# qianduoduolr/FGVC

Measured on AMD Instinct MI355X. Metric: frames/sec + ms/corr-volume, 480p 8-frame clip, 1/2/4/8 MI355X, higher is better.
Workload: dtype f16 + fp6 (e2m3) MFMA operands, f32 accumulate; top-k near-ties re-scored in f64 from f32 features

## Files before the change

### fgvc_amd/csrc/conv_split.hip

```cpp
#include "common.hpp"

namespace fgvc {

struct ConvSplitParams {
  const uint16_t* x;
  const uint16_t* w;
  const float* bias;
  const float* residual;
  uint16_t* y_split;
  float* y_f32;
  int N, H, W, Hp, Wp, Cin, Cout, relu;
  int n_ty, n_tx;
  int debug;
  float acc_scale;
  float out_scale;
  int out_fmt;
  int* overflow;
  const uint16_t* x2;
  const uint16_t* w2;
  int Cin2;
  unsigned char* y_bank;
  int bank_normalize;
  int bank_row_bytes;
};
// ... 730 lines not shown
__global__ __launch_bounds__(256) void normalize_nhwc_kernel(const float* __restrict__ in, float* __restrict__ out,
                                                              uint16_t* __restrict__ out_split, int C, int normalize,
                                                              long long npix) {
  const long long pixel = (long long)blockIdx.x * 4 + (threadIdx.x >> 6);
  const int lane = threadIdx.x & 63;
  if (pixel >= npix) return;
  const float* src = in + (size_t)pixel * C;
  float ss = 0.f;
  for (int c = lane * 4; c < C; c += 256) {
    const f32x4 v = *reinterpret_cast<const f32x4*>(src + c);
    ss += v.x * v.x + v.y * v.y + v.z * v.z + v.w * v.w;
  }
#pragma unroll
  for (int m = 32; m >= 1; m >>= 1) ss += __shfl_xor(ss, m);
  const float inv = normalize ? 1.0f / fmaxf(sqrtf(ss), 1e-12f) : 1.0f;
  for (int c = lane * 4; c < C; c += 256) {
    f32x4 v = *reinterpret_cast<const f32x4*>(src + c);
    v *= inv;
    if (out) *reinterpret_cast<f32x4*>(out + pixel * C + c) = v;
    if (out_split) {
      ushort4 hv, lv;
      if constexpr (FMT == 0) {
        split_bf16_4(v, hv, lv);
      } else {
        typedef _Float16 f16x4 __attribute__((ext_vector_type(4)));
        f16x4 h, l;
#pragma unroll
        for (int i = 0; i < 4; ++i) {
          const float xs = v[i] * 16384.f;
          h[i] = (_Float16)xs;
          l[i] = (_Float16)(xs - (float)h[i]);
        }
        hv = __builtin_bit_cast(ushort4, h);
        lv = __builtin_bit_cast(ushort4, l);
      }
      *reinterpret_cast<ushort4*>(out_split + pixel * 2 * C + c) = hv;
      *reinterpret_cast<ushort4*>(out_split + pixel * 2 * C + C + c) = lv;
    }
  }
}

__device__ __forceinline__ int n6_scale_exp(float m) {
  if (!(m > 0.f)) return -40;
  int e;
  const float f = frexpf(m * (1.0f / 7.5f), &e);
  int s = (f > 0.5f) ? e : e - 1;
  if (m * exp2f((float)-s) > 7.5f) ++s;
  return imax(s, -40);
}
__device__ __forceinline__ unsigned n6_code(float y) {
  const float a = fabsf(y);
  const float inv_step = a < 2.f ? 8.f : (a < 4.f ? 4.f : 2.f);
  const float r = fminf(__builtin_rintf(a * inv_step) / inv_step, 7.5f);
  const float c = r < 2.f ? 8.f * r : (r < 4.f ? 8.f + 4.f * r : 16.f + 2.f * r);
  return (unsigned)c | (y < 0.f ? 32u : 0u);
}
__global__ __launch_bounds__(256) void normalize_f16f6p_kernel(const float* __restrict__ in, unsigned char* __restrict__ out, int normalize,
                                                                long long npix, int rowb) {
  const long long pixel = (long long)blockIdx.x * 4 + (threadIdx.x >> 6);
  const int lane = threadIdx.x & 63;
  if (pixel >= npix) return;
  const float* src = in + (size_t)pixel * 256;
  float ss;
  {
#pragma clang fp contract(off)
    const f32x4 v = *reinterpret_cast<const f32x4*>(src + 4 * lane);
    const float xx = v.x * v.x, yy = v.y * v.y, zz = v.z * v.z, ww = v.w * v.w;
    ss = ((xx + yy) + zz) + ww;
  }
#pragma unroll
  for (int m = 32; m >= 1; m >>= 1) ss += __shfl_xor(ss, m);
  const float inv = normalize ? 1.0f / fmaxf(sqrtf(ss), 1e-12f) : 1.0f;
  f32x4 x = *reinterpret_cast<const f32x4*>(src + 4 * lane);
  x *= inv;
  unsigned char* row = out + (size_t)pixel * rowb;
  if (rowb > 1024) *reinterpret_cast<f32x4*>(row + 1024 + 16 * lane) = x;
  typedef _Float16 f16x4 __attribute__((ext_vector_type(4)));
  f16x4 hv;
  float hf[4], lf[4], mh = 0.f, ml = 0.f;
#pragma unroll
  for (int i = 0; i < 4; ++i) {
    const float xs = x[i] * 256.f;
    const _Float16 h = (_Float16)xs;
    hv[i] = h;
    hf[i] = (float)h;
    lf[i] = (xs - hf[i]) * 256.f;
    mh = fmaxf(mh, fabsf(hf[i]));
    ml = fmaxf(ml, fabsf(lf[i]));
  }
  *reinterpret_cast<f16x4*>(row + 8 * lane) = hv;
#pragma unroll
  for (int m = 1; m <= 8; m <<= 1) {
    if (m == 2) continue;
    mh = fmaxf(mh, __shfl_xor(mh, m));
    ml = fmaxf(ml, __shfl_xor(ml, m));
  }
  const int sh = n6_scale_exp(mh), sl = n6_scale_exp(ml);
  const float ih = exp2f((float)-sh), il = exp2f((float)-sl);
  unsigned ph = 0, pl = 0;
#pragma unroll
  for (int i = 0; i < 4; ++i) {
    ph |= n6_code(hf[i] * ih) << (6 * i);
    pl |= n6_code(lf[i] * il) << (6 * i);
  }
  const int v = lane >> 4, hi = (lane >> 1) & 1, pi = ((lane >> 2) & 3) * 2 + (lane & 1);
  const int w = pi < 6 ? pi : 0;
  const int pa = (4 * w) / 3, oa = 32 * w - 24 * pa;
  const int base = (lane & ~13) ;
  const int la = base + 4 * (pa >> 1) + (pa & 1), lb = base + 4 * ((pa + 1) >> 1) + ((pa + 1) & 1);
  const unsigned ha = __shfl(ph, la), hb = __shfl(ph, lb), qa = __shfl(pl, la), qb = __shfl(pl, lb);
  const unsigned wh = (ha >> oa) | (hb << (24 - oa)), wl = (qa >> oa) | (qb << (24 - oa));
  if (pi < 4) {
    *reinterpret_cast<unsigned*>(row + 512 + 32 * v + 16 * hi + 4 * pi) = wh;
    *reinterpret_cast<unsigned*>(row + 704 + 32 * v + 16 * hi + 4 * pi) = wl;
  } else if (pi < 6) {
    *reinterpret_cast<unsigned*>(row + 640 + 32 * (v >> 1) + 16 * hi + 8 * (v & 1) + 4 * (pi - 4)) = wh;
    *reinterpret_cast<unsigned*>(row + 832 + 32 * (v >> 1) + 16 * hi + 8 * (v & 1) + 4 * (pi - 4)) = wl;
  } else if (pi == 6) {
    row[896 + 16 * hi + v] = (unsigned char)(sh + 127 - 4);
  } else {
    row[896 + 16 * hi + 4 + v] = (unsigned char)(sl + 127 - 4);
  }
  if (lane < 2) *reinterpret_cast<unsigned long long*>(row + 904 + 16 * lane) = 0ull;
  else if (lane < 26) *reinterpret_cast<unsigned*>(row + 928 + 4 * (lane - 2)) = 0u;
}

static int g_conv_debug = 0;
void set_conv_debug(int v) { g_conv_debug = v; }
static int g_conv_narrow = 1;
void set_conv_narrow(int v) { g_conv_narrow = v; }
static int g_conv_cot_cap = 0;
void set_conv_cot_cap(int v) { g_conv_cot_cap = v; }

template <int COT, int OUT_FMT, bool RES, bool F32OUT, bool GENERIC, bool BANK = false, int CIN_TAG = 0>
__global__ __launch_bounds__(256, 1) void conv256p_kernel(ConvSplitParams p) {
  constexpr int NA = COT / 64, PPW = NA * 2;
  constexpr int TROWS = 8, PATCHB = (TROWS + 2) * CV_PW * 128, SLOTB = COT * 128, NPIECE = (TROWS + 2) * 5;
  __shared__ __attribute__((aligned(16))) unsigned char smem[PATCHB + 3 * SLOTB + COT * 4];
  unsigned char* patch = smem;
  unsigned char* wring = smem + PATCHB;
  float* bias_lds = reinterpret_cast<float*>(smem + PATCHB + 3 * SLOTB);
  const long long t_begin = __builtin_amdgcn_s_memtime();
  const int tid = threadIdx.x, lane = tid & 63;
  const int wave = __builtin_amdgcn_readfirstlane(tid >> 6);
  const int ch = wave & 1, pr = wave >> 1;
  const int n = lane & 31, h = lane >> 5;
  const int d_row = lane >> 3, d_slot = lane & 7;
  int bid = blockIdx.x;
  const int nimg = bid / (p.n_ty * p.n_tx);
  bid -= nimg * p.n_ty * p.n_tx;
  const int ty = bid / p.n_tx, tx = bid - ty * p.n_tx;
  const int y0 = ty * TROWS, x0 = tx * 32;
  const int co_base = blockIdx.y * COT;
  const int nchunk = p.Cin / 32;
  const uint32_t pixb = (uint32_t)nchunk * 128u;

  const uint32_t w_lane_off = (uint32_t)(d_row * 128 + ((d_slot ^ (d_row >> 1)) << 4));
  const uint32_t wo[2] = {w_lane_off, w_lane_off ^ 64u};
  const uint32_t ring_lds = lds_addr(wring), patch_lds = lds_addr(patch);
  const uint32_t wl = ring_lds + (uint32_t)((ch * (COT / 2) + n) * 128) + ((((uint32_t)h) ^ (uint32_t)((n >> 1) & 7)) << 4);
  uint32_t pl[3][2];
#pragma unroll
  for (int dx = 0; dx < 3; ++dx)
#pragma unroll
    for (int par = 0; par < 2; ++par) {
      const uint32_t key = (uint32_t)((((n + dx) >> 1) & 7) ^ (4 * par));
      pl[dx][par] = patch_lds + (uint32_t)((4 * pr * CV_PW + n + dx) * 128) + ((((uint32_t)h) ^ key) << 4);
    }
  const uint32_t pf_lane_off = (uint32_t)d_row * pixb + (uint32_t)((d_slot ^ (d_row >> 1)) << 4);
  const uint32_t lane16 = (uint32_t)lane * 16u;
  int ptab;
  {
    const int k = lane & 15, i = imin(wave + 4 * k, NPIECE - 1);
    const int prow = i / 5, pc0 = (i - prow * 5) * 8;
    const int goff = (int)((uint32_t)(prow * p.Wp + pc0) * pixb);
    const int ldst = (prow * CV_PW + pc0) * 128;
    const int key = ((prow + (pc0 >> 3)) & 1) << 6;
    ptab = lane < 16 ? goff : lane < 32 ? ldst : key;
  }
  const unsigned char* xb_tile = reinterpret_cast<const unsigned char*>(p.x) + (uint32_t)((nimg * p.Hp + y0) * p.Wp + x0) * pixb;
  const unsigned char* wb_tile = reinterpret_cast<const unsigned char*>(p.w) + (uint32_t)(co_base * 128);
  const uint32_t piece_off = (uint32_t)(wave * PPW * 1024);
  auto weight_base = [&](int chunk, int tap) { return wb_tile + (uint32_t)((tap * nchunk + chunk) * p.Cout * 128); };
  auto weight_piece = [&](const unsigned char* base, uint32_t dst, int j) {
    const unsigned char* src = base + piece_off + (uint32_t)(j * 1024);
    const uint32_t d = dst + piece_off + (uint32_t)(j * 1024);
    asm volatile("s_mov_b32 m0, %2\n\ts_nop 0\n\tglobal_load_lds_dwordx4 %0, %1" ::"v"(wo[j & 1]), "s"(src), "s"(d) : "memory");
  };

  if (tid < COT / 4) reinterpret_cast<f32x4*>(bias_lds)[tid] = reinterpret_cast<const f32x4*>(p.bias + co_base)[tid];
  for (int i = wave; i < NPIECE; i += 4) {
    const int prow = i / 5, pc0 = (i - prow * 5) * 8;
    const int P = prow * CV_PW + pc0 + d_row;
    const int sl = d_slot ^ ((P >> 1) & 7);
    const size_t gpix = ((size_t)nimg * p.Hp + (y0 + prow)) * p.Wp + (x0 + pc0 + d_row);
    conv_lds_dma_16(reinterpret_cast<const unsigned char*>(p.x) + gpix * pixb + sl * 16, lds_addr(patch + (prow * CV_PW + pc0) * 128));
  }
#pragma unroll
  for (int j = 0; j < PPW; ++j) weight_piece(weight_base(0, 0), ring_lds, j);
#pragma unroll
  for (int j = 0; j < PPW; ++j) weight_piece(weight_base(0, 1), ring_lds + SLOTB, j);

  __builtin_amdgcn_s_waitcnt(0x0F70);

  const long long t_loop0 = __builtin_amdgcn_s_memtime();
  {
    const size_t wb64 = (size_t)wb_tile, xb64 = (size_t)xb_tile;
    const int s_tap = __builtin_amdgcn_readfirstlane(nchunk * p.Cout * 128), s_chunk = __builtin_amdgcn_readfirstlane(p.Cout * 128);
    const int s_nchunk = __builtin_amdgcn_readfirstlane(nchunk), s_ring = __builtin_amdgcn_readfirstlane((int)ring_lds);
    const int s_patch = __builtin_amdgcn_readfirstlane((int)patch_lds), s_piece = __builtin_amdgcn_readfirstlane((int)piece_off);
    typedef int i32x2 __attribute__((ext_vector_type(2)));
    const i32x2 s_wb = {__builtin_amdgcn_readfirstlane((int)(uint32_t)wb64), __builtin_amdgcn_readfirstlane((int)(uint32_t)(wb64 >> 32))};
    const i32x2 s_xb = {__builtin_amdgcn_readfirstlane((int)(uint32_t)xb64), __builtin_amdgcn_readfirstlane((int)(uint32_t)(xb64 >> 32))};
    typedef int i32x2_t __attribute__((ext_vector_type(2)));
    i32x2_t loop_cycles;
    const int nchunk2 = p.x2 ? p.Cin2 / 32 : 0;
    const uint32_t pixb2 = (uint32_t)nchunk2 * 128u;
    const uint32_t pf_lane_off2 = (uint32_t)d_row * pixb2 + (uint32_t)((d_slot ^ (d_row >> 1)) << 4);
    int ptab2;
    {
      const int k2 = lane & 15, i2 = imin(wave + 4 * k2, NPIECE - 1);
      const int prow = i2 / 5, pc0 = (i2 - prow * 5) * 8;
      const int goff = (int)((uint32_t)(prow * p.Wp + pc0) * pixb2);
      ptab2 = lane < 16 ? goff : lane < 32 ? (prow * CV_PW + pc0) * 128 : (((prow + (pc0 >> 3)) & 1) << 6);
    }
    const size_t w2b64 = (size_t)p.w2 + (uint32_t)(co_base * 128), x2b64 = (size_t)p.x2 + (size_t)((uint32_t)((nimg * p.Hp + y0) * p.Wp + x0) * pixb2);
    const i32x2 s_w2b = {__builtin_amdgcn_readfirstlane((int)(uint32_t)w2b64), __builtin_amdgcn_readfirstlane((int)(uint32_t)(w2b64 >> 32))};
    const i32x2 s_x2b = {__builtin_amdgcn_readfirstlane((int)(uint32_t)x2b64), __builtin_amdgcn_readfirstlane((int)(uint32_t)(x2b64 >> 32))};
    const int s_last2 = __builtin_amdgcn_readfirstlane(nchunk2 ? nchunk - 1 : -1), s_nchunk2 = __builtin_amdgcn_readfirstlane(nchunk2);
#define C256P_INPUTS                                                                                                              \
  "{v232}"(wl), "{v233}"(pl[0][0]), "{v234}"(pl[0][1]), "{v235}"(pl[1][0]), "{v236}"(pl[1][1]), "{v237}"(pl[2][0]), "{v238}"(pl[2][1]),     \
      "{v239}"(wo[0]), "{v240}"(wo[1]), "{v241}"(pf_lane_off), "{v242}"(lane16), "{v243}"(ptab), "{v244}"(pf_lane_off2), "{v245}"(ptab2),  \
      "{s[20:21]}"(s_wb), "{s22}"(s_tap), "{s23}"(s_chunk), "{s[24:25]}"(s_xb), "{s26}"(s_nchunk), "{s27}"(s_ring), "{s28}"(s_patch),      \
      "{s29}"(s_piece), "{s46}"(s_last2), "{s[48:49]}"(s_w2b), "{s[50:51]}"(s_x2b), "{s52}"(s_nchunk2)
    if constexpr (COT == 256) {
#include "conv256p_loop.inc"
    } else {
#include "conv128p_loop.inc"
    }
#undef C256P_INPUTS
    if ((p.debug & 8) && blockIdx.x == 300 && blockIdx.y == 0 && lane == 0 && p.y_split) {
      long long* o = reinterpret_cast<long long*>(p.y_split) + wave * 8;
      o[4] = (long long)(uint32_t)loop_cycles.x | ((long long)loop_cycles.y << 32);
      o[5] = nchunk * 9 + nchunk2;
      o[0] = t_loop0 - t_begin;
    }
  }
  f32x16 acc[NA][4];
  if constexpr (NA == 4)
    asm volatile(""
                 : "={a[0:15]}"(acc[0][0]), "={a[16:31]}"(acc[0][1]), "={a[32:47]}"(acc[0][2]), "={a[48:63]}"(acc[0][3]), "={a[64:79]}"(acc[1][0]),
                   "={a[80:95]}"(acc[1][1]), "={a[96:111]}"(acc[1][2]), "={a[112:127]}"(acc[1][3]), "={a[128:143]}"(acc[NA - 2][0]),
                   "={a[144:159]}"(acc[NA - 2][1]), "={a[160:175]}"(acc[NA - 2][2]), "={a[176:191]}"(acc[NA - 2][3]), "={a[192:207]}"(acc[NA - 1][0]),
                   "={a[208:223]}"(acc[NA - 1][1]), "={a[224:239]}"(acc[NA - 1][2]), "={a[240:255]}"(acc[NA - 1][3]));
  else
    asm volatile(""
                 : "={a[0:15]}"(acc[0][0]), "={a[16:31]}"(acc[0][1]), "={a[32:47]}"(acc[0][2]), "={a[48:63]}"(acc[0][3]), "={a[64:79]}"(acc[1][0]),
                   "={a[80:95]}"(acc[1][1]), "={a[96:111]}"(acc[1][2]), "={a[112:127]}"(acc[1][3]));

  int lane_e;
  asm volatile("v_mbcnt_lo_u32_b32 %0, -1, 0\n\tv_mbcnt_hi_u32_b32 %0, -1, %0" : "=v"(lane_e));
  {
  int lane = lane_e, n = lane & 31, h = lane >> 5;
  int Wp_e = __builtin_amdgcn_readfirstlane(p.Wp);
  asm volatile("" : "+s"(Wp_e));
  constexpr int RPW = 4, CW = COT / 2, RB = CW * 4, RS = RB + 16, LPR = RB / 16, RPI = 64 / LPR;
  static_assert(4 * 32 * RS <= PATCHB + 3 * SLOTB, "epilogue staging");
  __syncthreads();
  long long ts0 = __builtin_amdgcn_s_memtime(), ts1 = 0, ts2 = 0, ts3 = 0, ts4 = 0;
  unsigned char* tile = smem + wave * (32 * RS);
  const int co_w = co_base + ch * CW;
  int mv_row = lane / LPR, mv_col = (lane % LPR) * 16;
  auto row_fence = [&]() { asm volatile("" : "+v"(n), "+v"(h), "+v"(mv_row), "+v"(mv_col)); };
  auto wave_sync = [&]() { asm volatile("s_waitcnt lgkmcnt(0)" ::: "memory"); };
  constexpr int RSLOTS = RB / 16, RPIECES = 32 * RB / 1024, RPPP = 1024 / RB;
  static_assert(4 * 32 * RS + 4 * 32 * RB <= PATCHB + 3 * SLOTB, "residual tiles");
  unsigned char* rtile = smem + 4 * (32 * RS) + wave * (32 * RB);
  const bool has_res = GENERIC || BANK ? p.residual != nullptr : RES;
  auto residual_dma = [&](int b_) {
    const int y_ = y0 + RPW * pr + b_;
    if (!has_res || b_ >= RPW || y_ >= p.H) return;
    const unsigned char* src = reinterpret_cast<const unsigned char*>(p.residual + (((size_t)nimg * p.H + y_) * p.W + x0) * p.Cout + co_w);
    const int pmax = p.W - 1 - x0;
#pragma unroll
    for (int j = 0; j < RPIECES; ++j) {
      const int pp = j * RPPP + (lane * 16) / RB, ps = ((lane * 16) % RB) / 16;
      const uint32_t voff = (uint32_t)(imin(pp, pmax) * p.Cout * 4 + ((ps ^ (pp & (RSLOTS - 1))) << 4));
      conv_lds_dma_16s(voff, src, lds_addr(rtile + j * 1024));
    }
  };
  auto residual_wait = [&](int stores_behind) {
    if (x0 + 32 > p.W || stores_behind == 0) asm volatile("s_waitcnt vmcnt(0)" ::: "memory");
    else if (stores_behind == 32 / RPI) asm volatile("s_waitcnt vmcnt(%0)" ::"n"(32 / RPI) : "memory");
    else asm volatile("s_waitcnt vmcnt(%0)" ::"n"(2 * (32 / RPI)) : "memory");
  };
  auto residual_at = [&](int cw) {
    return *reinterpret_cast<const f32x4*>(rtile + n * RB + ((((cw * 4) >> 4) ^ (n & (RSLOTS - 1))) << 4));
  };
  residual_dma(0);
  const bool tile_full = x0 + 32 <= p.W;
  auto store_rows = [&](unsigned char* dst) {
    unsigned char* d0 = dst + (size_t)mv_row * p.Cout * 4 + mv_col;
    const unsigned char* t0 = tile + mv_row * RS + mv_col;
    if (tile_full) {
#pragma unroll
      for (int i = 0; i < 32 / RPI; ++i) *reinterpret_cast<uint4*>(d0 + (size_t)(i * RPI) * p.Cout * 4) = *reinterpret_cast<const uint4*>(t0 + i * RPI * RS);
    } else {
#pragma unroll
      for (int i = 0; i < 32 / RPI; ++i)
        if (x0 + i * RPI + mv_row < p.W) *reinterpret_cast<uint4*>(d0 + (size_t)(i * RPI) * p.Cout * 4) = *reinterpret_cast<const uint4*>(t0 + i * RPI * RS);
    }
  };
  if constexpr (BANK) {
    {
      constexpr int BK_RS = 1024 + 16;
      static_assert(COT == 256 && 2 * 32 * BK_RS <= PATCHB + 3 * SLOTB, "bank staging");
      unsigned char* rows = smem + pr * (32 * BK_RS);
      float* part = reinterpret_cast<float*>(rows);
      long long bts[6] = {}, bt_begin = 0;
#pragma unroll
      for (int b = 0; b < RPW; ++b) {
        row_fence();
        const int y = y0 + RPW * pr + b;
        const bool row_ok = y < p.H;
        if (b == 1) bt_begin = __builtin_amdgcn_s_memtime();
        if (b == 2) bts[4] = __builtin_amdgcn_s_memtime();
        const size_t fpix0 = ((size_t)nimg * p.H + imin(y, p.H - 1)) * p.W + x0;
        if (has_res && row_ok) residual_wait(b == 0 || 32 / RPI != 16 ? 0 : (p.bank_row_bytes > 1024 ? 32 : 16));
        f32x4 v[NA][4];
#pragma unroll
        for (int a = 0; a < NA; ++a)
#pragma unroll
          for (int g = 0; g < 4; ++g) {
            const int cw = a * 32 + 8 * g + 4 * h;
            const f32x4 bv = *reinterpret_cast<const f32x4*>(bias_lds + ch * CW + cw);
            v[a][g] = {fmaf(acc[a][b][4 * g + 0], p.acc_scale, bv.x), fmaf(acc[a][b][4 * g + 1], p.acc_scale, bv.y),
                         fmaf(acc[a][b][4 * g + 2], p.acc_scale, bv.z), fmaf(acc[a][b][4 * g + 3], p.acc_scale, bv.w)};
            if (has_res && row_ok) v[a][g] += residual_at(cw);
            if (p.relu) {
              v[a][g].x = fmaxf(v[a][g].x, 0.f); v[a][g].y = fmaxf(v[a][g].y, 0.f);
              v[a][g].z = fmaxf(v[a][g].z, 0.f); v[a][g].w = fmaxf(v[a][g].w, 0.f);
            }
          }
        if (has_res) { wave_sync(); residual_dma(b + 1); }
        if (b == 1) bts[0] = __builtin_amdgcn_s_memtime();
        __syncthreads();
        float pp[NA][4];
        {
#pragma clang fp contract(off)
#pragma unroll
          for (int a = 0; a < NA; ++a)
#pragma unroll
            for (int g = 0; g < 4; ++g) {
              const float xx = v[a][g].x * v[a][g].x, yy = v[a][g].y * v[a][g].y, zz = v[a][g].z * v[a][g].z, ww = v[a][g].w * v[a][g].w;
              pp[a][g] = ((xx + yy) + zz) + ww;
              part[(ch * 16 + a * 4 + g) * 64 + lane] = pp[a][g];
            }
        }
        __syncthreads();
        float ss;
        {
          float t[NA][4];
#pragma unroll
          for (int a = 0; a < NA; ++a)
#pragma unroll
            for (int g = 0; g < 4; ++g) t[a][g] = pp[a][g] + part[((ch ^ 1) * 16 + a * 4 + g) * 64 + lane];
          float u[2][4], w4[4];
#pragma unroll
          for (int g = 0; g < 4; ++g) { u[0][g] = t[0][g] + t[2][g]; u[1][g] = t[1][g] + t[3][g]; }
#pragma unroll
          for (int g = 0; g < 4; ++g) w4[g] = u[0][g] + u[1][g];
          const float z0 = w4[0] + w4[2], z1 = w4[1] + w4[3];
          const float s1 = z0 + z1;
          ss = s1 + __shfl_xor(s1, 32);
        }
        __syncthreads();
        if (b == 1) bts[1] = __builtin_amdgcn_s_memtime();
        const float inv = p.bank_normalize ? 1.0f / fmaxf(sqrtf(ss), 1e-12f) : 1.0f;
        unsigned char* row = rows + n * BK_RS;
#pragma unroll
        for (int vl = 0; vl < 2; ++vl)
#pragma unroll
          for (int hi = 0; hi < 2; ++hi) {
            unsigned A_[16], B_[16];
            float mh = 0.f, ml = 0.f;
#pragma unroll
            for (int m = 0; m < 4; ++m) {
              const int a = 2 * vl + (m >> 1), g = hi + 2 * (m & 1);
              f32x4 x = v[a][g];
              x *= inv;
              typedef _Float16 f16x4 __attribute__((ext_vector_type(4)));
              f16x4 hv;
#pragma unroll
              for (int k = 0; k < 4; ++k) {
                const float xs = x[k] * 256.f;
                const _Float16 hh_ = (_Float16)xs;
                hv[k] = hh_;
                const float fh = (float)hh_, fl = (xs - fh) * 256.f;
                mh = fmaxf(mh, fabsf(fh)); ml = fmaxf(ml, fabsf(fl));
                A_[4 * m + k] = __builtin_bit_cast(unsigned, fh);
                B_[4 * m + k] = __builtin_bit_cast(unsigned, fl);
              }
              *reinterpret_cast<f16x4*>(row + 2 * (128 * ch + 32 * a + 8 * g + 4 * h)) = hv;
            }
#pragma unroll
            for (int j = 0; j < 16; ++j) {
              const auto t2 = __builtin_amdgcn_permlane32_swap(A_[j], B_[j], false, false);
              A_[j] = t2[0]; B_[j] = t2[1];
            }
            const auto tm = __builtin_amdgcn_permlane32_swap(__builtin_bit_cast(unsigned, mh), __builtin_bit_cast(unsigned, ml), false, false);
            const unsigned mb = tm[0] > tm[1] ? tm[0] : tm[1];
            int sexp = (int)(mb >> 23) - 129 + ((mb & 0x7fffffu) > 0x700000u ? 1 : 0);
            sexp = (mb == 0u || sexp < -40) ? -40 : sexp;
            fgvc_i32x16 S0, S1;
#pragma unroll
            for (int m = 0; m < 4; ++m) {
              S0[4 * m + 0] = (int)A_[4 * m + 0]; S0[4 * m + 1] = (int)A_[4 * m + 2]; S0[4 * m + 2] = (int)B_[4 * m + 0]; S0[4 * m + 3] = (int)B_[4 * m + 2];
              S1[4 * m + 0] = (int)A_[4 * m + 1]; S1[4 * m + 1] = (int)A_[4 * m + 3]; S1[4 * m + 2] = (int)B_[4 * m + 1]; S1[4 * m + 3] = (int)B_[4 * m + 3];
            }
            fgvc_i32x6 c6;
            const unsigned sc_bits = (unsigned)(sexp + 127) << 23;
            asm volatile("v_cvt_scalef32_2xpk16_fp6_f32 %0, %1, %2, %3" : "=&v"(c6) : "v"(S0), "v"(S1), "v"(sc_bits));
            const int vg = 2 * ch + vl;
            *reinterpret_cast<i32x4*>(row + (h ? 704 : 512) + 32 * vg + 16 * hi) = i32x4{c6[0], c6[1], c6[2], c6[3]};
            *reinterpret_cast<uint2*>(row + (h ? 832 : 640) + 32 * (vg >> 1) + 16 * hi + 8 * (vg & 1)) = uint2{(unsigned)c6[4], (unsigned)c6[5]};
            row[896 + 16 * hi + 4 * h + vg] = (unsigned char)(sexp + 127 - 4);
          }
        if (ch == 0) {
          if (h == 0) {
            *reinterpret_cast<unsigned long long*>(row + 904) = 0ull;
            *reinterpret_cast<unsigned long long*>(row + 920) = 0ull;
          } else {
#pragma unroll
            for (int i = 0; i < 6; ++i) *reinterpret_cast<i32x4*>(row + 928 + 16 * i) = i32x4{0, 0, 0, 0};
          }
        }
        if (b == 1) bts[2] = __builtin_amdgcn_s_memtime();
        __syncthreads();
        if (row_ok) {
          unsigned char* dst = p.y_bank + fpix0 * p.bank_row_bytes;
          if (x0 + 32 <= p.W) {
#pragma unroll
            for (int i = 0; i < 16; ++i) {
              const int r = 16 * ch + i;
              *reinterpret_cast<uint4*>(dst + (size_t)r * p.bank_row_bytes + 16 * lane) = *reinterpret_cast<const uint4*>(rows + r * BK_RS + 16 * lane);
            }
          } else {
#pragma unroll
            for (int i = 0; i < 16; ++i) {
              const int r = 16 * ch + i;
              if (x0 + r < p.W)
                *reinterpret_cast<uint4*>(dst + (size_t)r * p.bank_row_bytes + 16 * lane) = *reinterpret_cast<const uint4*>(rows + r * BK_RS + 16 * lane);
            }
          }
        }
        __syncthreads();
        if (b == 1) bts[3] = __builtin_amdgcn_s_memtime();
        if (p.bank_row_bytes > 1024) {
#pragma unroll
          for (int a = 0; a < NA; ++a)
#pragma unroll
            for (int g = 0; g < 4; ++g) {
              f32x4 x = v[a][g];
              x *= inv;
              *reinterpret_cast<f32x4*>(row + 4 * (128 * ch + 32 * a + 8 * g + 4 * h)) = x;
            }
          __syncthreads();
          if (row_ok) {
            unsigned char* dst = p.y_bank + fpix0 * p.bank_row_bytes + 1024;
            if (x0 + 32 <= p.W) {
#pragma unroll
              for (int i = 0; i < 16; ++i) {
                const int r = 16 * ch + i;
                *reinterpret_cast<uint4*>(dst + (size_t)r * p.bank_row_bytes + 16 * lane) = *reinterpret_cast<const uint4*>(rows + r * BK_RS + 16 * lane);
              }
            } else {
#pragma unroll
              for (int i = 0; i < 16; ++i) {
                const int r = 16 * ch + i;
                if (x0 + r < p.W)
                  *reinterpret_cast<uint4*>(dst + (size_t)r * p.bank_row_bytes + 16 * lane) = *reinterpret_cast<const uint4*>(rows + r * BK_RS + 16 * lane);
              }
            }
          }
          __syncthreads();
        }
      }
      if ((p.debug & 8) && blockIdx.x == 300 && blockIdx.y == 0 && lane == 0) {
        long long* o_ = reinterpret_cast<long long*>(p.y_bank) + wave * 8;
        o_[0] = bts[0] - bt_begin; o_[1] = bts[1] - bts[0]; o_[2] = bts[2] - bts[1]; o_[3] = bts[3] - bts[2]; o_[4] = bts[4] - bts[3]; o_[5] = __builtin_amdgcn_s_memtime() - t_begin;
      }
      return;
    }
  }
  constexpr bool HOIST_BIAS = false;
  constexpr bool FUSE_RELU = !GENERIC && !F32OUT && OUT_FMT == 3;
  const float clamp_lo = __builtin_bit_cast(float, __builtin_amdgcn_readfirstlane(FUSE_RELU && p.relu ? 0 : (int)0xC77FE000u));
  f32x4 bvv[HOIST_BIAS ? NA : 1][4];
  if constexpr (HOIST_BIAS) {
#pragma unroll
    for (int a = 0; a < NA; ++a)
#pragma unroll
      for (int g = 0; g < 4; ++g) bvv[a][g] = *reinterpret_cast<const f32x4*>(bias_lds + ch * CW + a * 32 + 8 * g + 4 * h);
  }
#pragma unroll
  for (int b = 0; b < RPW; ++b) {
    row_fence();
    const int y = y0 + RPW * pr + b;
    if (y >= p.H) continue;
    const size_t pix0 = ((size_t)nimg * p.Hp + (y + 1)) * Wp_e + (x0 + 1);
    const size_t fpix0 = ((size_t)nimg * p.H + y) * p.W + x0;
    if (has_res) residual_wait(b == 0 ? 0 : ((GENERIC ? p.y_f32 != nullptr : F32OUT) ? 32 / RPI : 0) + (p.y_split ? 32 / RPI : 0));
    f32x4 v[NA][4];
#pragma unroll
    for (int a = 0; a < NA; ++a)
#pragma unroll
      for (int g = 0; g < 4; ++g) {
        const int cw = a * 32 + 8 * g + 4 * h;
        const f32x4 bv = HOIST_BIAS ? bvv[HOIST_BIAS ? a : 0][g] : *reinterpret_cast<const f32x4*>(bias_lds + ch * CW + cw);
        v[a][g] = {fmaf(acc[a][b][4 * g + 0], p.acc_scale, bv.x), fmaf(acc[a][b][4 * g + 1], p.acc_scale, bv.y),
                   fmaf(acc[a][b][4 * g + 2], p.acc_scale, bv.z), fmaf(acc[a][b][4 * g + 3], p.acc_scale, bv.w)};
        if (has_res) v[a][g] += residual_at(cw);
        if (p.relu && !FUSE_RELU) {
          v[a][g].x = fmaxf(v[a][g].x, 0.f); v[a][g].y = fmaxf(v[a][g].y, 0.f);
          v[a][g].z = fmaxf(v[a][g].z, 0.f); v[a][g].w = fmaxf(v[a][g].w, 0.f);
        }
      }
    if (has_res) { wave_sync(); residual_dma(b + 1); }
    if (b == 1) { asm volatile("s_nop 0" ::"v"(v[0][0]), "v"(v[3][3])); ts1 = __builtin_amdgcn_s_memtime(); }
    if (GENERIC ? p.y_f32 != nullptr : F32OUT) {
      wave_sync();
#pragma unroll
      for (int a = 0; a < NA; ++a)
#pragma unroll
        for (int g = 0; g < 4; ++g) *reinterpret_cast<f32x4*>(tile + n * RS + (a * 32 + 8 * g + 4 * h) * 4) = v[a][g];
      wave_sync();
      store_rows(reinterpret_cast<unsigned char*>(p.y_f32 + fpix0 * p.Cout + co_w));
    }
    if (p.y_split) {
      wave_sync();
      const int out_fmt = GENERIC ? p.out_fmt : OUT_FMT;
      if (out_fmt == 0) {
#pragma unroll
        for (int a = 0; a < NA; ++a)
#pragma unroll
          for (int g = 0; g < 4; ++g) {
            ushort4 hv, lv;
            split_bf16_4(v[a][g], hv, lv);
            unsigned char* o = tile + n * RS + a * 128 + (8 * g + 4 * h) * 2;
            *reinterpret_cast<ushort4*>(o) = hv;
            *reinterpret_cast<ushort4*>(o + 64) = lv;
          }
      } else if (out_fmt == 3) {
        bool ovf = false;
#pragma unroll
        for (int a = 0; a < NA; ++a) {
          uint2 hw[4];
          i32x4 main6, tail6;
          split_f16f6_chunk(v[a], p.out_scale, h, hw, main6, tail6, ovf, clamp_lo);
          unsigned char* o = tile + n * RS + a * 128;
#pragma unroll
          for (int g = 0; g < 4; ++g) *reinterpret_cast<uint2*>(o + (8 * g + 4 * h) * 2) = hw[g];
          *reinterpret_cast<i32x4*>(o + 80 - 16 * h) = main6;
          *reinterpret_cast<i32x4*>(o + 112 - 16 * h) = tail6;
        }
        if (__builtin_amdgcn_ballot_w64(ovf && x0 + n < p.W) != 0ull && lane == 0) atomicOr(p.overflow, 1);
      } else {
        bool ovf = false;
#pragma unroll
        for (int a = 0; a < NA; ++a)
#pragma unroll
          for (int g = 0; g < 4; ++g) {
            uint2 hw, lw;
            uint32_t l8, h8;
            split_f16_4(v[a][g], p.out_scale, hw, l8, h8, lw, ovf);
            unsigned char* o = tile + n * RS + a * 128;
            *reinterpret_cast<uint2*>(o + (8 * g + 4 * h) * 2) = hw;
            if (out_fmt == 1) {
              *reinterpret_cast<uint32_t*>(o + 64 + 8 * g + 4 * h) = l8;
              *reinterpret_cast<uint32_t*>(o + 96 + 8 * g + 4 * h) = h8;
            } else {
              *reinterpret_cast<uint2*>(o + 64 + (8 * g + 4 * h) * 2) = lw;
            }
          }
        if (__builtin_amdgcn_ballot_w64(ovf && x0 + n < p.W) != 0ull && lane == 0) atomicOr(p.overflow, 1);
      }
      wave_sync();
      if (b == 1) ts2 = __builtin_amdgcn_s_memtime();
      store_rows(reinterpret_cast<unsigned char*>(p.y_split) + (pix0 * (p.Cout / 32) + (co_w >> 5)) * 128);
    }
    wave_sync();
    if (b == 0) ts4 = __builtin_amdgcn_s_memtime();
    if (b == 1) ts3 = __builtin_amdgcn_s_memtime();
  }
  if ((p.debug & 8) && blockIdx.x == 300 && blockIdx.y == 0 && lane == 0 && p.y_split) {
    long long* o_ = reinterpret_cast<long long*>(p.y_split) + wave * 8;
    o_[2] = ts4 - ts0; o_[3] = ts1 - ts4; o_[6] = ts2 - ts1; o_[7] = ts3 - ts2;
    asm volatile("s_waitcnt vmcnt(0)" ::: "memory");
    reinterpret_cast<long long*>(p.y_split)[wave * 8 + 1] = __builtin_amdgcn_s_memtime() - t_begin;
  }
  }
}

template <int ARITH>
static void conv_split_dispatch(const ConvSplitParams& p, dim3 grid, int KS, int cot_eff, bool narrow, hipStream_t s) {
  if (KS == 3) {
    if (cot_eff == 256 && p.y_bank) conv_split_kernel<3, 256, 1, 3, 4, false, ARITH, 2, true><<<grid, 512, 0, s>>>(p);
    else if (cot_eff == 256 && p.x2) conv_split_kernel<3, 256, 1, 3, 4, false, ARITH, 2, false, true><<<grid, 512, 0, s>>>(p);
    else if (cot_eff == 256) conv_split_kernel<3, 256, 1, 3, 4, false, ARITH><<<grid, 512, 0, s>>>(p);
    else if (cot_eff == 128 && narrow) conv_split_kernel<3, 128, 1, 3, 2, false, ARITH><<<grid, 256, 0, s>>>(p);
    else if (cot_eff == 128) conv_split_kernel<3, 128, 3, 2, 4, false, ARITH><<<grid, 512, 0, s>>>(p);
    else if (narrow) conv_split_kernel<3, 64, 3, 2, 2, false, ARITH><<<grid, 256, 0, s>>>(p);
    else conv_split_kernel<3, 64, 3, 3, 4, false, ARITH><<<grid, 512, 0, s>>>(p);
  } else {
    if (cot_eff == 256) conv_split_kernel<1, 256, 1, 3, 4, false, ARITH><<<grid, 512, 0, s>>>(p);
    else if (cot_eff == 128) conv_split_kernel<1, 128, 1, 3, 4, false, ARITH><<<grid, 512, 0, s>>>(p);
    else if (narrow) conv_split_kernel<1, 64, 1, 3, 2, false, ARITH><<<grid, 256, 0, s>>>(p);
    else conv_split_kernel<1, 64, 1, 3, 4, false, ARITH><<<grid, 512, 0, s>>>(p);
  }
}

int conv_split_launch(const uint16_t* x, const uint16_t* w, const float* bias, const float* residual, uint16_t* y_split,
                      float* y_f32, int N, int H, int W, int Hp, int Wp, int Cin, int Cout, int KS, int relu, int in_fmt,
                      int in_scale_log2, int out_fmt, int out_scale_log2, int* overflow, hipStream_t s, unsigned char* y_bank,
                      int bank_normalize, const uint16_t* x2, const uint16_t* w2, int Cin2, int bank_row_bytes) {
  ConvSplitParams p;
  p.x = x; p.w = w; p.bias = bias; p.residual = residual; p.y_split = y_split; p.y_f32 = y_f32;
  p.N = N; p.H = H; p.W = W; p.Hp = Hp; p.Wp = Wp; p.Cin = Cin; p.Cout = Cout; p.relu = relu;
  p.acc_scale = ldexpf(1.0f, -in_scale_log2); p.out_scale = ldexpf(1.0f, out_scale_log2); p.out_fmt = out_fmt; p.overflow = overflow;
  p.y_bank = y_bank; p.bank_normalize = bank_normalize; p.bank_row_bytes = bank_row_bytes;
  p.x2 = x2; p.w2 = w2; p.Cin2 = Cin2;
  const int cot = (Cout % 256 == 0) ? 256 : (Cout % 128 == 0) ? 128 : 64;
  const int cot_eff = (g_conv_cot_cap && cot > g_conv_cot_cap && !y_bank && !x2) ? g_conv_cot_cap : cot;
  const bool narrow = (cot_eff == 64 && (g_conv_narrow & 1)) || (cot_eff == 128 && KS == 3 && (g_conv_narrow & 2));
  p.n_ty = cdiv(H, narrow ? 4 : 8); p.n_tx = cdiv(W, 32);
  p.debug = g_conv_debug;
  dim3 grid(p.n_ty * p.n_tx * N, Cout / cot_eff);
  const bool fits32 = (unsigned long long)N * Hp * Wp * (Cin / 32) * 128ull < (1ull << 32) && (unsigned long long)9 * Cin * Cout * 4ull < (1ull << 32) &&
                      (!x2 || ((unsigned long long)N * Hp * Wp * (Cin2 / 32) * 128ull < (1ull << 32) && (unsigned long long)Cin2 * Cout * 4ull < (1ull << 32)));
  if (in_fmt == 3 && KS == 3 && (cot_eff == 256 || cot_eff == 128) && !narrow && (!y_bank || (cot_eff == 256 && !x2)) && (!x2 || (cot_eff == 256 && Cin2 >= 32)) &&
      Cin >= 32 && fits32 && !(g_conv_debug & 1024)) {
    if (y_bank) conv256p_kernel<256, -1, false, false, true, true><<<grid, 256, 0, s>>>(p);
    else if (cot_eff == 256) {
      if (y_split && out_fmt == 3 && !residual && !y_f32 && p.Cin == 128) conv256p_kernel<256, 3, false, false, false, false, 1><<<grid, 256, 0, s>>>(p);
      else if (y_split && out_fmt == 3 && !residual && !y_f32) conv256p_kernel<256, 3, false, false, false><<<grid, 256, 0, s>>>(p);
      else if (y_split && out_fmt == 3 && !residual && y_f32) conv256p_kernel<256, 3, false, true, false><<<grid, 256, 0, s>>>(p);
      else if (y_split && out_fmt == 3 && residual && y_f32) conv256p_kernel<256, 3, true, true, false><<<grid, 256, 0, s>>>(p);
      else if (y_split && out_fmt == 3 && residual && !y_f32) conv256p_kernel<256, 3, true, false, false><<<grid, 256, 0, s>>>(p);
      else conv256p_kernel<256, -1, false, false, true><<<grid, 256, 0, s>>>(p);
    } else {
      if (y_split && out_fmt == 3 && !residual && !y_f32) conv256p_kernel<128, 3, false, false, false><<<grid, 256, 0, s>>>(p);
      else if (y_split && out_fmt == 3 && residual && y_f32) conv256p_kernel<128, 3, true, true, false><<<grid, 256, 0, s>>>(p);
      else if (y_split && out_fmt == 3 && residual && !y_f32) conv256p_kernel<128, 3, true, false, false><<<grid, 256, 0, s>>>(p);
      else conv256p_kernel<128, -1, false, false, true><<<grid, 256, 0, s>>>(p);
    }
    FGVC_CHECK_LAUNCH("fgvc_conv_split_f32");
    return FGVC_OK;
  }
  if (in_fmt == 1) conv_split_dispatch<1>(p, grid, KS, cot_eff, narrow, s);
  else if (in_fmt == 3) conv_split_dispatch<3>(p, grid, KS, cot_eff, narrow, s);
  else if (in_fmt == 2) conv_split_dispatch<2>(p, grid, KS, cot_eff, narrow, s);
  else if (KS == 3 && cot_eff == 256 && !(g_conv_debug & 16) && !y_bank && !x2) conv_split_kernel<3, 256, 1, 3, 4, true><<<grid, 512, 0, s>>>(p);
  else conv_split_dispatch<0>(p, grid, KS, cot_eff, narrow, s);
  FGVC_CHECK_LAUNCH("fgvc_conv_split_f32");
  return FGVC_OK;
}

int nchw_to_split_nhwc_launch(const float* in, uint16_t* out, float* out_f32, int N, int C, int H, int W, int Hp, int Wp,
                              hipStream_t s) {
  dim3 grid(cdiv(W, 256), H, N * (C / 32));
  nchw_to_split_nhwc_kernel<<<grid, 256, 0, s>>>(in, out, out_f32, C, H, W, Hp, Wp);
  FGVC_CHECK_LAUNCH("fgvc_nchw_to_split_nhwc_f32");
  return FGVC_OK;
}

__global__ __launch_bounds__(256) void nhwc_to_split_kernel(float* __restrict__ x, uint16_t* __restrict__ out, int C, int H,
                                                             int W, int Hp, int Wp, int relu, long long n_vec4) {
  const long long g = (long long)blockIdx.x * 256 + threadIdx.x;
  if (g >= n_vec4) return;
  const long long e = g * 4;
  const long long pixel = e / C;
  const int c = (int)(e - pixel * C);
  const int nimg = (int)(pixel / ((long long)H * W));
  const int rem = (int)(pixel - (long long)nimg * H * W);
  const int y = rem / W, xx = rem - y * W;
  f32x4 v = *reinterpret_cast<const f32x4*>(x + e);
  if (relu) {
    v.x = fmaxf(v.x, 0.f); v.y = fmaxf(v.y, 0.f); v.z = fmaxf(v.z, 0.f); v.w = fmaxf(v.w, 0.f);
    *reinterpret_cast<f32x4*>(x + e) = v;
  }
  ushort4 hv, lv;
  split_bf16_4(v, hv, lv);
  uint16_t* o = out + ((((size_t)nimg * Hp + (y + 1)) * Wp + (xx + 1)) * (C / 32) + (c >> 5)) * 64 + (c & 31);
  *reinterpret_cast<ushort4*>(o) = hv;
  *reinterpret_cast<ushort4*>(o + 32) = lv;
}

int nhwc_to_split_launch(float* x, uint16_t* out, int N, int C, int H, int W, int Hp, int Wp, int relu, hipStream_t s) {
  const long long n4 = (long long)N * H * W * C / 4;
  nhwc_to_split_kernel<<<(unsigned)((n4 + 255) / 256), 256, 0, s>>>(x, out, C, H, W, Hp, Wp, relu, n4);
  FGVC_CHECK_LAUNCH("fgvc_nhwc_to_split_f32");
  return FGVC_OK;
}

int normalize_nhwc_launch(const float* in, float* out, uint16_t* out_split, int N, int C, int H, int W, int normalize,
                          int split_fmt, hipStream_t s) {
  const long long npix = (long long)N * H * W;
  if (split_fmt == 2 || split_fmt == 3)
    normalize_f16f6p_kernel<<<(unsigned)((npix + 3) / 4), 256, 0, s>>>(in, reinterpret_cast<unsigned char*>(out_split), normalize, npix, split_fmt == 3 ? 2048 : 1024);
  else if (split_fmt == 0) normalize_nhwc_kernel<0><<<(unsigned)((npix + 3) / 4), 256, 0, s>>>(in, out, out_split, C, normalize, npix);
  else normalize_nhwc_kernel<1><<<(unsigned)((npix + 3) / 4), 256, 0, s>>>(in, out, out_split, C, normalize, npix);
  FGVC_CHECK_LAUNCH("fgvc_normalize_nhwc_f32");
  return FGVC_OK;
}

}
```

Before: 2056.

## Pipeline conv epilogue stores through double-buffered LDS staging and batch LDS reads

```diff
diff --git a/fgvc_amd/csrc/conv_split.hip b/fgvc_amd/csrc/conv_split.hip
--- a/fgvc_amd/csrc/conv_split.hip
+++ b/fgvc_amd/csrc/conv_split.hip
@@ -1056,13 +1056,17 @@
   auto store_rows = [&](unsigned char* dst) {
     unsigned char* d0 = dst + (size_t)mv_row * p.Cout * 4 + mv_col;
     const unsigned char* t0 = tile + mv_row * RS + mv_col;
+    i32x4 rb[32 / RPI];
+#pragma unroll
+    for (int i = 0; i < 32 / RPI; ++i) rb[i] = *reinterpret_cast<const i32x4*>(t0 + i * RPI * RS);
+    __builtin_amdgcn_sched_barrier(0);
     if (tile_full) {
 #pragma unroll
-      for (int i = 0; i < 32 / RPI; ++i) *reinterpret_cast<uint4*>(d0 + (size_t)(i * RPI) * p.Cout * 4) = *reinterpret_cast<const uint4*>(t0 + i * RPI * RS);
+      for (int i = 0; i < 32 / RPI; ++i) *reinterpret_cast<i32x4*>(d0 + (size_t)(i * RPI) * p.Cout * 4) = rb[i];
     } else {
 #pragma unroll
       for (int i = 0; i < 32 / RPI; ++i)
-        if (x0 + i * RPI + mv_row < p.W) *reinterpret_cast<uint4*>(d0 + (size_t)(i * RPI) * p.Cout * 4) = *reinterpret_cast<const uint4*>(t0 + i * RPI * RS);
+        if (x0 + i * RPI + mv_row < p.W) *reinterpret_cast<i32x4*>(d0 + (size_t)(i * RPI) * p.Cout * 4) = rb[i];
     }
   };
   if constexpr (BANK) {
@@ -1072,6 +1076,20 @@
       unsigned char* rows = smem + pr * (32 * BK_RS);
       float* part = reinterpret_cast<float*>(rows);
       long long bts[6] = {}, bt_begin = 0;
+      auto bank_store = [&](unsigned char* dst) {
+        i32x4 rb[16];
+#pragma unroll
+        for (int i = 0; i < 16; ++i) rb[i] = *reinterpret_cast<const i32x4*>(rows + (16 * ch + i) * BK_RS + 16 * lane);
+        __builtin_amdgcn_sched_barrier(0);
+        if (x0 + 32 <= p.W) {
+#pragma unroll
+          for (int i = 0; i < 16; ++i) *reinterpret_cast<i32x4*>(dst + (size_t)(16 * ch + i) * p.bank_row_bytes + 16 * lane) = rb[i];
+        } else {
+#pragma unroll
+          for (int i = 0; i < 16; ++i)
+            if (x0 + 16 * ch + i < p.W) *reinterpret_cast<i32x4*>(dst + (size_t)(16 * ch + i) * p.bank_row_bytes + 16 * lane) = rb[i];
+        }
+      };
 #pragma unroll
       for (int b = 0; b < RPW; ++b) {
         row_fence();
@@ -1191,23 +1209,7 @@
         }
         if (b == 1) bts[2] = __builtin_amdgcn_s_memtime();
         __syncthreads();
-        if (row_ok) {
-          unsigned char* dst = p.y_bank + fpix0 * p.bank_row_bytes;
-          if (x0 + 32 <= p.W) {
-#pragma unroll
-            for (int i = 0; i < 16; ++i) {
-              const int r = 16 * ch + i;
-              *reinterpret_cast<uint4*>(dst + (size_t)r * p.bank_row_bytes + 16 * lane) = *reinterpret_cast<const uint4*>(rows + r * BK_RS + 16 * lane);
-            }
-          } else {
-#pragma unroll
-            for (int i = 0; i < 16; ++i) {
-              const int r = 16 * ch + i;
-              if (x0 + r < p.W)
-                *reinterpret_cast<uint4*>(dst + (size_t)r * p.bank_row_bytes + 16 * lane) = *reinterpret_cast<const uint4*>(rows + r * BK_RS + 16 * lane);
-            }
-          }
-        }
+        if (row_ok) bank_store(p.y_bank + fpix0 * p.bank_row_bytes);
         __syncthreads();
         if (b == 1) bts[3] = __builtin_amdgcn_s_memtime();
         if (p.bank_row_bytes > 1024) {
@@ -1220,23 +1222,7 @@
               *reinterpret_cast<f32x4*>(row + 4 * (128 * ch + 32 * a + 8 * g + 4 * h)) = x;
             }
           __syncthreads();
-          if (row_ok) {
-            unsigned char* dst = p.y_bank + fpix0 * p.bank_row_bytes + 1024;
-            if (x0 + 32 <= p.W) {
-#pragma unroll
-              for (int i = 0; i < 16; ++i) {
-                const int r = 16 * ch + i;
-                *reinterpret_cast<uint4*>(dst + (size_t)r * p.bank_row_bytes + 16 * lane) = *reinterpret_cast<const uint4*>(rows + r * BK_RS + 16 * lane);
-              }
-            } else {
-#pragma unroll
-              for (int i = 0; i < 16; ++i) {
-                const int r = 16 * ch + i;
-                if (x0 + r < p.W)
-                  *reinterpret_cast<uint4*>(dst + (size_t)r * p.bank_row_bytes + 16 * lane) = *reinterpret_cast<const uint4*>(rows + r * BK_RS + 16 * lane);
-              }
-            }
-          }
+          if (row_ok) bank_store(p.y_bank + fpix0 * p.bank_row_bytes + 1024);
           __syncthreads();
         }
       }
@@ -1257,6 +1243,115 @@
 #pragma unroll
       for (int g = 0; g < 4; ++g) bvv[a][g] = *reinterpret_cast<const f32x4*>(bias_lds + ch * CW + a * 32 + 8 * g + 4 * h);
   }
+  constexpr bool PIPE = !GENERIC && !RES && OUT_FMT == 3;
+  if constexpr (PIPE) {
+    static_assert(2 * 4 * 32 * RS <= PATCHB + 3 * SLOTB, "two staging sets");
+    constexpr int NS = 32 / RPI, PER = NS / NA;
+    static_assert(NS % NA == 0, "a staged row leaves in NA parts");
+    auto fence = [&]() { asm volatile("" ::: "memory"); __builtin_amdgcn_sched_barrier(0); };
+    const unsigned char* pend_t = nullptr;
+    unsigned char* pend_d = nullptr;
+    i32x4 rb[PER];
+    auto drain_read = [&](int q) {
+#pragma unroll
+      for (int i = 0; i < PER; ++i) rb[i] = *reinterpret_cast<const i32x4*>(pend_t + (q * PER + i) * RPI * RS);
+    };
+    auto drain_store = [&](int q) {
+      if (tile_full) {
+#pragma unroll
+        for (int i = 0; i < PER; ++i) *reinterpret_cast<i32x4*>(pend_d + (size_t)((q * PER + i) * RPI) * p.Cout * 4) = rb[i];
+      } else {
+#pragma unroll
+        for (int i = 0; i < PER; ++i)
+          if (x0 + (q * PER + i) * RPI + mv_row < p.W) *reinterpret_cast<i32x4*>(pend_d + (size_t)((q * PER + i) * RPI) * p.Cout * 4) = rb[i];
+      }
+    };
+    constexpr int NF = F32OUT ? 2 : 1;
+#pragma unroll
+    for (int b = 0; b < RPW; ++b) {
+      row_fence();
+      const int y = y0 + RPW * pr + b;
+      if (y >= p.H) break;
+      const size_t pix0 = ((size_t)nimg * p.Hp + (y + 1)) * Wp_e + (x0 + 1);
+      f32x4 v[NA][4], bvr[NA][4];
+#pragma unroll
+      for (int a = 0; a < NA; ++a)
+#pragma unroll
+        for (int g = 0; g < 4; ++g) bvr[a][g] = *reinterpret_cast<const f32x4*>(bias_lds + ch * CW + a * 32 + 8 * g + 4 * h);
+      __builtin_amdgcn_sched_barrier(0);
+#pragma unroll
+      for (int a = 0; a < NA; ++a)
+#pragma unroll
+        for (int g = 0; g < 4; ++g) {
+          const f32x4 bv = bvr[a][g];
+          v[a][g] = {fmaf(acc[a][b][4 * g + 0], p.acc_scale, bv.x), fmaf(acc[a][b][4 * g + 1], p.acc_scale, bv.y),
+                     fmaf(acc[a][b][4 * g + 2], p.acc_scale, bv.z), fmaf(acc[a][b][4 * g + 3], p.acc_scale, bv.w)};
+          if (p.relu && !FUSE_RELU) {
+            v[a][g].x = fmaxf(v[a][g].x, 0.f); v[a][g].y = fmaxf(v[a][g].y, 0.f);
+            v[a][g].z = fmaxf(v[a][g].z, 0.f); v[a][g].w = fmaxf(v[a][g].w, 0.f);
+          }
+        }
+      if (b == 1) { asm volatile("s_nop 0" ::"v"(v[0][0]), "v"(v[NA - 1][3])); ts1 = __builtin_amdgcn_s_memtime(); }
+      if constexpr (F32OUT) {
+        const size_t fpix0 = ((size_t)nimg * p.H + y) * p.W + x0;
+        unsigned char* cur = smem + (((NF * b) & 1) * 4 + wave) * (32 * RS);
+#pragma unroll
+        for (int a = 0; a < NA; ++a) {
+          fence();
+          if (b > 0) drain_read(a);
+          fence();
+#pragma unroll
+          for (int g = 0; g < 4; ++g) *reinterpret_cast<f32x4*>(cur + n * RS + (a * 32 + 8 * g + 4 * h) * 4) = v[a][g];
+          fence();
+          if (b > 0) drain_store(a);
+        }
+        fence();
+        pend_t = cur + mv_row * RS + mv_col;
+        pend_d = reinterpret_cast<unsigned char*>(p.y_f32 + fpix0 * p.Cout + co_w) + (size_t)mv_row * p.Cout * 4 + mv_col;
+      }
+      {
+        unsigned char* cur = smem + (((NF * b + NF - 1) & 1) * 4 + wave) * (32 * RS);
+        bool ovf = false;
+#pragma unroll
+        for (int a = 0; a < NA; ++a) {
+          fence();
+          if (b > 0 || F32OUT) drain_read(a);
+          fence();
+          uint2 hw[4];
+          i32x4 main6, tail6;
+          split_f16f6_chunk(v[a], p.out_scale, h, hw, main6, tail6, ovf, clamp_lo);
+          unsigned char* o = cur + n * RS + a * 128;
+#pragma unroll
+          for (int g = 0; g < 4; ++g) *reinterpret_cast<uint2*>(o + (8 * g + 4 * h) * 2) = hw[g];
+          *reinterpret_cast<i32x4*>(o + 80 - 16 * h) = main6;
+          *reinterpret_cast<i32x4*>(o + 112 - 16 * h) = tail6;
+          fence();
+          if (b > 0 || F32OUT) drain_store(a);
+        }
+        fence();
+        if (__builtin_amdgcn_ballot_w64(ovf && x0 + n < p.W) != 0ull && lane == 0) atomicOr(p.overflow, 1);
+        pend_t = cur + mv_row * RS + mv_col;
+        pend_d = reinterpret_cast<unsigned char*>(p.y_split) + (pix0 * (p.Cout / 32) + (co_w >> 5)) * 128 + (size_t)mv_row * p.Cout * 4 + mv_col;
+      }
+      if (b == 0) ts4 = __builtin_amdgcn_s_memtime();
+      if (b == 1) ts2 = ts3 = __builtin_amdgcn_s_memtime();
+    }
+    fence();
+    if (pend_t != nullptr) {
+      i32x4 rl[NS];
+#pragma unroll
+      for (int i = 0; i < NS; ++i) rl[i] = *reinterpret_cast<const i32x4*>(pend_t + i * RPI * RS);
+      __builtin_amdgcn_sched_barrier(0);
+      if (tile_full) {
+#pragma unroll
+        for (int i = 0; i < NS; ++i) *reinterpret_cast<i32x4*>(pend_d + (size_t)(i * RPI) * p.Cout * 4) = rl[i];
+      } else {
+#pragma unroll
+        for (int i = 0; i < NS; ++i)
+          if (x0 + i * RPI + mv_row < p.W) *reinterpret_cast<i32x4*>(pend_d + (size_t)(i * RPI) * p.Cout * 4) = rl[i];
+      }
+    }
+  } else {
 #pragma unroll
   for (int b = 0; b < RPW; ++b) {
     row_fence();
@@ -1265,16 +1360,27 @@
     const size_t pix0 = ((size_t)nimg * p.Hp + (y + 1)) * Wp_e + (x0 + 1);
     const size_t fpix0 = ((size_t)nimg * p.H + y) * p.W + x0;
     if (has_res) residual_wait(b == 0 ? 0 : ((GENERIC ? p.y_f32 != nullptr : F32OUT) ? 32 / RPI : 0) + (p.y_split ? 32 / RPI : 0));
-    f32x4 v[NA][4];
+    f32x4 v[NA][4], bvr[GENERIC ? 1 : NA][4], rvr[GENERIC ? 1 : NA][4];
+    if constexpr (!GENERIC) {
+#pragma unroll
+      for (int a = 0; a < NA; ++a)
+#pragma unroll
+        for (int g = 0; g < 4; ++g) {
+          const int cw = a * 32 + 8 * g + 4 * h;
+          bvr[a][g] = HOIST_BIAS ? bvv[HOIST_BIAS ? a : 0][g] : *reinterpret_cast<const f32x4*>(bias_lds + ch * CW + cw);
+          if (has_res) rvr[a][g] = residual_at(cw);
+        }
+      __builtin_amdgcn_sched_barrier(0);
+    }
 #pragma unroll
     for (int a = 0; a < NA; ++a)
 #pragma unroll
       for (int g = 0; g < 4; ++g) {
         const int cw = a * 32 + 8 * g + 4 * h;
-        const f32x4 bv = HOIST_BIAS ? bvv[HOIST_BIAS ? a : 0][g] : *reinterpret_cast<const f32x4*>(bias_lds + ch * CW + cw);
+        const f32x4 bv = !GENERIC ? bvr[GENERIC ? 0 : a][g] : HOIST_BIAS ? bvv[HOIST_BIAS ? a : 0][g] : *reinterpret_cast<const f32x4*>(bias_lds + ch * CW + cw);
         v[a][g] = {fmaf(acc[a][b][4 * g + 0], p.acc_scale, bv.x), fmaf(acc[a][b][4 * g + 1], p.acc_scale, bv.y),
                    fmaf(acc[a][b][4 * g + 2], p.acc_scale, bv.z), fmaf(acc[a][b][4 * g + 3], p.acc_scale, bv.w)};
-        if (has_res) v[a][g] += residual_at(cw);
+        if (has_res) v[a][g] += GENERIC ? residual_at(cw) : rvr[GENERIC ? 0 : a][g];
         if (p.relu && !FUSE_RELU) {
           v[a][g].x = fmaxf(v[a][g].x, 0.f); v[a][g].y = fmaxf(v[a][g].y, 0.f);
           v[a][g].z = fmaxf(v[a][g].z, 0.f); v[a][g].w = fmaxf(v[a][g].w, 0.f);
@@ -1346,6 +1452,7 @@
     wave_sync();
     if (b == 0) ts4 = __builtin_amdgcn_s_memtime();
     if (b == 1) ts3 = __builtin_amdgcn_s_memtime();
+  }
   }
   if ((p.debug & 8) && blockIdx.x == 300 && blockIdx.y == 0 && lane == 0 && p.y_split) {
     long long* o_ = reinterpret_cast<long long*>(p.y_split) + wave * 8;
```

After: 2061, median of 3. Within noise of the previous version (+0.2%).
